# gaetanfacchinetti/DensityFlows.jl

Measured on AMD Instinct MI355X. Metric: forward+logdetJ Msamples/s, d=5 8-layer RealNVP, 1/2/4/8 MI355X, higher is better.
Workload: dtype f32

## Files before the change

densityflows.jl_amd/csrc/df_chain_impl.h:

```cpp
#pragma once

#include <hip/hip_runtime.h>

#include "df_kernels.h"

namespace df {

typedef float f32x4 __attribute__((ext_vector_type(4)));

#ifndef DF_WAVES_PER_EU
#define DF_WAVES_PER_EU(HT) ((HT) <= 4 ? 4 : 2)
#endif

namespace impl {

__device__ __forceinline__ float relu(float x) {
    return __int_as_float(__builtin_elementwise_max(__float_as_int(x), 0));
}

__device__ __forceinline__ float tanh_fast(float x) {
    const float x2 = x * x;
    const float n = fmaf(fmaf(fmaf(fmaf(1.587199e-8f, x2, 2.2332108e-5f), x2, 0.0035974074f), x2, 0.1346604f), x2, 1.0f);
    const float d =
        fmaf(fmaf(fmaf(fmaf(8.7767893e-7f, x2, 0.0003453992f), x2, 0.026262015f), x2, 0.4679937f), x2, 1.0f);
    return (x2 < 66.f) ? x * (n / d) : (x > 0.f ? 1.f : (x < 0.f ? -1.f : x));
}

__device__ __forceinline__ float sigmoid_fast(float x) {
    const float t = expf(-fabsf(x));
    const float y = (x >= 0.f) ? 1.f / (1.f + t) : t / (1.f + t);
    return (x > 40.f) ? 1.f : ((x < -80.f) ? 0.f : y);
}

__device__ __noinline__ float act_fn(int act, float x) {
    switch (act) {
        case DF_ACT_IDENTITY: return x;
        case DF_ACT_RELU: return relu(x);
        case DF_ACT_TANH: return tanh_fast(x);
        case DF_ACT_SIGMOID: return sigmoid_fast(x);
        case DF_ACT_SOFTPLUS: return log1pf(expf(-fabsf(x))) + ((x > 0.f) ? x : 0.f);
        case DF_ACT_LOGCOSH: {
            float y = -2.f * x;
            float sp = log1pf(expf(-fabsf(y))) + ((y > 0.f) ? y : 0.f);
            return (x + sp) - 0.6931471805599453f;
        }
        case DF_ACT_LEAKYRELU: return (x > 0.f) ? x : 0.01f * x;
        case DF_ACT_ELU: return (x > 0.f) ? x : expm1f(x);
        case DF_ACT_SWISH: {
            float t = expf(-fabsf(x));
            float sg = (x >= 0.f) ? 1.f / (1.f + t) : t / (1.f + t);
            return x * sg;
        }
        default: return x;
    }
}

__device__ __forceinline__ f32x4 mfma4(float a, float b, f32x4 c) {
    return __builtin_amdgcn_mfma_f32_16x16x4f32(a, b, c, 0, 0, 0);
}

__device__ __forceinline__ f32x4 lds4(const uint8_t* p) { return *reinterpret_cast<const f32x4*>(p); }

struct Smem {
    const int32_t* tab;
    float* state;
};

struct Stager {
    uint8_t* base;
    int bytes;
    const int32_t* sched;
    int n;
    int idx;
    int cur;
    __device__ __forceinline__ uint8_t* buf() const { return base + ((idx & 1) ? bytes : 0); }
};

template <typename T>
__device__ __forceinline__ T cload(const T* p, int64_t i) {
    using CT = const __attribute__((address_space(4))) T;
    return *(const T*)(&((CT*)(uintptr_t)p)[i]);
}

__device__ __forceinline__ void dma_stage(const ChainArgs& a, int s, uint8_t* dst) {
    const DevStage st = cload(a.stages, s);
    const int wave = __builtin_amdgcn_readfirstlane(threadIdx.x >> 6), lane = threadIdx.x & 63;
    const uint8_t* src = a.blob + st.src_off;
    const int nchunk = st.bytes >> 10;
    for (int c = wave; c < nchunk; c += kWavesPerBlock) {
        __builtin_amdgcn_global_load_lds(reinterpret_cast<const void*>(src + (c << 10) + lane * 16),
                                         (__attribute__((address_space(3))) void*)(dst + (c << 10)),
                                         16, 0, 0);
    }
}

__device__ __forceinline__ void stager_start(Stager& sg, const ChainArgs& a) {
    sg.idx = -1;
    sg.cur = -1;
    if (sg.n > 0) dma_stage(a, cload(sg.sched, 0), sg.base);
}

__device__ __forceinline__ void ensure_stage(int s, Stager& sg, const ChainArgs& a) {
    if (s == sg.cur) return;
#ifdef DF_EXP_NOSYNC
    if (sg.cur >= 0) { sg.cur = s; return; }
#endif
    const int nidx = sg.idx + 1;
    asm volatile("s_waitcnt vmcnt(0)" ::: "memory");
    __syncthreads();
    sg.idx = nidx;
    sg.cur = s;
    if (nidx >= sg.n || cload(sg.sched, nidx) != s) {
        const DevStage st = cload(a.stages, s);
        const f32x4* src = reinterpret_cast<const f32x4*>(a.blob + st.src_off);
        f32x4* dst = reinterpret_cast<f32x4*>(sg.buf());
        for (int i = threadIdx.x; i < (st.bytes >> 4); i += kBlockThreads) dst[i] = src[i];
        __syncthreads();
        sg.n = 0;
        return;
    }
    if (nidx + 1 < sg.n) dma_stage(a, cload(sg.sched, nidx + 1), sg.base + (((nidx + 1) & 1) ? sg.bytes : 0));
}

constexpr int out_tiles(int HT) { return HT < 2 ? HT : 2; }

template <int HT, int T, bool OUTV>
struct NetRegs {
    f32x4 h[T][HT];
    f32x4 acc[T][HT];
    f32x4 out[T][OUTV ? 1 : out_tiles(HT)];
};

template <int HT, int T>
__device__ __forceinline__ void dense_mfma(const ChainArgs& a, const DevDense& D, const int32_t* feat,
                                           Stager& sg, const Smem& sm, const int (&rowoff)[T],
                                           f32x4 (&h)[T][HT], f32x4 (&acc)[T][HT]) {
    const int lane = threadIdx.x & 63;
    const int g = lane >> 4;
    constexpr int MG = (T == 1) ? 2 : 1;
#pragma unroll
    for (int tt = 0; tt < T; ++tt)
#pragma unroll
        for (int m = 0; m < HT; ++m) acc[tt][m] = f32x4{0.f, 0.f, 0.f, 0.f};

    for (int c = 0; c < D.n_chunks; ++c) {
        const DevChunk C = a.chunks[D.chunk0 + c];
        ensure_stage(C.stage, sg, a);
        const uint8_t* base = sg.buf() + C.lds_off + lane * 16;
        if (D.in_kind == IN_STATE) {
#pragma unroll
            for (int kq = 0; kq < kMaxState / 16; ++kq) {
                if (kq >= C.kq_begin && kq < C.kq_end) {
                    float xin[T][4];
#pragma unroll
                    for (int r = 0; r < 4; ++r) {
                        const int s = 4 * kq + r;
                        if (s < D.ks) {
                            const int slot = feat[4 * s + g];
#pragma unroll
                            for (int tt = 0; tt < T; ++tt) xin[tt][r] = sm.state[rowoff[tt] + slot];
                        } else {
#pragma unroll
                            for (int tt = 0; tt < T; ++tt) xin[tt][r] = 0.f;
                        }
                    }
                    const uint8_t* bq = base + (kq - C.kq_begin) * D.mt * 1024;
                    if (HT >= 8 && D.mt == HT) {
                        constexpr int MB = HT < 4 ? HT : 4;
                        const int rmax = D.ks - 4 * kq;
#pragma unroll
                        for (int m0 = 0; m0 < HT; m0 += MB) {
                            f32x4 w[MB];
#pragma unroll
                            for (int mm = 0; mm < MB; ++mm) w[mm] = lds4(bq + (m0 + mm) * 1024);
#pragma unroll
                            for (int r = 0; r < 4; ++r)
                                if (r < rmax)
#pragma unroll
                                    for (int mm = 0; mm < MB; ++mm)
#pragma unroll
                                        for (int tt = 0; tt < T; ++tt)
                                            acc[tt][m0 + mm] = mfma4(w[mm][r], xin[tt][r], acc[tt][m0 + mm]);
                        }
                        continue;
                    }
#pragma unroll
                    for (int m0 = 0; m0 < HT; m0 += MG) {
                        if (m0 < D.mt) {
                            f32x4 w[MG];
#pragma unroll
                            for (int mm = 0; mm < MG; ++mm)
                                w[mm] = (m0 + mm < D.mt) ? lds4(bq + (m0 + mm) * 1024) : f32x4{0, 0, 0, 0};
#pragma unroll
                            for (int r = 0; r < 4; ++r) {
                                if (4 * kq + r < D.ks) {
#pragma unroll
                                    for (int mm = 0; mm < MG; ++mm)
                                        if (m0 + mm < HT && m0 + mm < D.mt)
#pragma unroll
                                            for (int tt = 0; tt < T; ++tt)
                                                acc[tt][m0 + mm] = mfma4(w[mm][r], xin[tt][r], acc[tt][m0 + mm]);
                                }
                            }
                        }
                    }
                }
            }
        } else if (D.mt == HT && C.kq_begin == 0 && C.kq_end == HT) {
            constexpr int MB = HT < 4 ? HT : 4;
#pragma unroll
            for (int m0 = 0; m0 < HT; m0 += MB) {
                f32x4 w[2][MB];
#pragma unroll
                for (int mm = 0; mm < MB; ++mm) w[0][mm] = lds4(base + (m0 + mm) * 1024);
#pragma unroll
                for (int kq = 0; kq < HT; ++kq) {
                    const int cb = kq & 1;
                    if (kq + 1 < HT) {
#pragma unroll
                        for (int mm = 0; mm < MB; ++mm)
                            w[cb ^ 1][mm] = lds4(base + ((kq + 1) * HT + m0 + mm) * 1024);
                    }
#pragma unroll
                    for (int r = 0; r < 4; ++r)
#pragma unroll
                        for (int mm = 0; mm < MB; ++mm)
#pragma unroll
                            for (int tt = 0; tt < T; ++tt)
                                acc[tt][m0 + mm] = mfma4(w[cb][mm][r], h[tt][kq][r], acc[tt][m0 + mm]);
                }
            }
        } else if (HT >= 8 && D.mt <= 2) {
            const int kb = C.kq_begin, ke = C.kq_end;
#pragma unroll
            for (int kq = 0; kq < HT; ++kq) {
                if (kq >= kb && kq < ke) {
                    const uint8_t* bq = base + (kq - kb) * D.mt * 1024;
                    const f32x4 w0 = lds4(bq);
                    if (D.mt == 2) {
                        const f32x4 w1 = lds4(bq + 1024);
#pragma unroll
                        for (int r = 0; r < 4; ++r)
#pragma unroll
                            for (int tt = 0; tt < T; ++tt) {
                                acc[tt][0] = mfma4(w0[r], h[tt][kq][r], acc[tt][0]);
                                acc[tt][1] = mfma4(w1[r], h[tt][kq][r], acc[tt][1]);
                            }
                    } else {
#pragma unroll
                        for (int r = 0; r < 4; ++r)
#pragma unroll
                            for (int tt = 0; tt < T; ++tt) acc[tt][0] = mfma4(w0[r], h[tt][kq][r], acc[tt][0]);
                    }
                }
            }
        } else if (D.mt == HT) {
            constexpr int MB = HT < 4 ? HT : 4;
            const int kb = C.kq_begin, ke = C.kq_end;
#pragma unroll
            for (int kq = 0; kq < HT; ++kq) {
                if (kq >= kb && kq < ke) {
                    const uint8_t* bq = base + (kq - kb) * HT * 1024;
                    f32x4 w[2][MB];
#pragma unroll
                    for (int mm = 0; mm < MB; ++mm) w[0][mm] = lds4(bq + mm * 1024);
#pragma unroll
                    for (int m0 = 0; m0 < HT; m0 += MB) {
                        const int cb = (m0 / MB) & 1;
                        if (m0 + MB < HT) {
#pragma unroll
                            for (int mm = 0; mm < MB; ++mm) w[cb ^ 1][mm] = lds4(bq + (m0 + MB + mm) * 1024);
                        }
#pragma unroll
                        for (int r = 0; r < 4; ++r)
#pragma unroll
                            for (int mm = 0; mm < MB; ++mm)
#pragma unroll
                                for (int tt = 0; tt < T; ++tt)
                                    acc[tt][m0 + mm] = mfma4(w[cb][mm][r], h[tt][kq][r], acc[tt][m0 + mm]);
                    }
                }
            }
        } else {
#pragma unroll
            for (int kq = 0; kq < HT; ++kq) {
                if (kq >= C.kq_begin && kq < C.kq_end) {
                    const uint8_t* bq = base + (kq - C.kq_begin) * D.mt * 1024;
#pragma unroll
                    for (int m0 = 0; m0 < HT; m0 += MG) {
                        if (m0 < D.mt) {
                            f32x4 w[MG];
#pragma unroll
                            for (int mm = 0; mm < MG; ++mm)
                                w[mm] = (m0 + mm < D.mt) ? lds4(bq + (m0 + mm) * 1024) : f32x4{0, 0, 0, 0};
#pragma unroll
                            for (int r = 0; r < 4; ++r)
#pragma unroll
                                for (int mm = 0; mm < MG; ++mm)
                                    if (m0 + mm < HT && m0 + mm < D.mt)
#pragma unroll
                                        for (int tt = 0; tt < T; ++tt)
                                            acc[tt][m0 + mm] = mfma4(w[mm][r], h[tt][kq][r], acc[tt][m0 + mm]);
                        }
                    }
                }
            }
        }
    }

    ensure_stage(D.bias_stage, sg, a);
    if (D.has_bias) {
#pragma unroll
        for (int m = 0; m < HT; ++m) {
            if (m < D.mt) {
                const f32x4 b = lds4(sg.buf() + D.bias_lds + ((16 * m + 4 * g) << 2));
#pragma unroll
                for (int tt = 0; tt < T; ++tt) acc[tt][m] = acc[tt][m] + b;
            }
        }
    }
    if (D.act == DF_ACT_RELU) {
#pragma unroll
        for (int m = 0; m < HT; ++m)
#pragma unroll
            for (int tt = 0; tt < T; ++tt)
#pragma unroll
                for (int r = 0; r < 4; ++r) acc[tt][m][r] = relu(acc[tt][m][r]);
    } else if (D.act != DF_ACT_IDENTITY) {
#ifndef DF_NO_GENERIC_ACT
#pragma unroll
        for (int m = 0; m < HT; ++m) {
            if (m < D.mt) {
#pragma unroll
                for (int tt = 0; tt < T; ++tt)
#pragma unroll
                    for (int r = 0; r < 4; ++r) acc[tt][m][r] = act_fn(D.act, acc[tt][m][r]);
            }
        }
#endif
    }
}

template <int HT, int T, bool OUTV>
__device__ __forceinline__ void eval_net(const ChainArgs& a, const DevLayer& L, int dense0, int ndense,
                                         Stager& sg, const Smem& sm, const int (&rowoff)[T],
                                         NetRegs<HT, T, OUTV>& R, float* hs = nullptr, int64_t gs = -1) {
    const int lane = threadIdx.x & 63;
    const int g = lane >> 4;
    const int32_t* feat = sm.tab + L.feat_tab;
    for (int k = 0; k < ndense; ++k) {
        const DevDense D = a.denses[dense0 + k];
        if (OUTV && k + 1 == ndense) {
            ensure_stage(D.w3_stage, sg, a);
            const uint8_t* w3 = sg.buf() + D.w3_lds;
            const int inp = 16 * D.kt_in;
            const float* b3 = reinterpret_cast<const float*>(w3) + D.n_out * inp;
#pragma unroll
            for (int o = 0; o < 4; ++o) {
                if (o < D.n_out) {
                    float p[T];
#pragma unroll
                    for (int tt = 0; tt < T; ++tt) p[tt] = 0.f;
#pragma unroll
                    for (int kq = 0; kq < HT; ++kq) {
                        if (kq < D.kt_in) {
                            f32x4 w = lds4(w3 + ((o * inp + 16 * kq + 4 * g) << 2));
#pragma unroll
                            for (int r = 0; r < 4; ++r)
#pragma unroll
                                for (int tt = 0; tt < T; ++tt) p[tt] = __builtin_fmaf(w[r], R.h[tt][kq][r], p[tt]);
                        }
                    }
#pragma unroll
                    for (int tt = 0; tt < T; ++tt) {
                        p[tt] += __shfl_xor(p[tt], 16);
                        p[tt] += __shfl_xor(p[tt], 32);
                        float v = p[tt];
                        if (D.has_bias) v = v + b3[o];
                        R.out[tt][0][o] = (D.act == DF_ACT_IDENTITY) ? v : act_fn(D.act, v);
                    }
                } else {
#pragma unroll
                    for (int tt = 0; tt < T; ++tt) R.out[tt][0][o] = 0.f;
                }
            }
            return;
        }
        dense_mfma<HT, T>(a, D, feat, sg, sm, rowoff, R.h, R.acc);
        if (k + 1 == ndense) {
            if constexpr (!OUTV) {
#pragma unroll
                for (int tt = 0; tt < T; ++tt)
#pragma unroll
                    for (int m = 0; m < out_tiles(HT); ++m) R.out[tt][m] = R.acc[tt][m];
            }
        } else {
#pragma unroll
            for (int tt = 0; tt < T; ++tt)
#pragma unroll
                for (int m = 0; m < HT; ++m) R.h[tt][m] = R.acc[tt][m];
            if (hs && gs >= 0) {
                float* dst = hs + ((int64_t)k * a.batch + gs) * a.hsave_w + 4 * g;
#pragma unroll
                for (int m = 0; m < HT; ++m)
                    if (m < D.mt) *reinterpret_cast<f32x4*>(dst + 16 * m) = R.acc[0][m];
            }
        }
    }
}

__device__ __forceinline__ float sel4(const f32x4 v, int i) {
    float r = v[0];
    r = (i == 1) ? v[1] : r;
    r = (i == 2) ? v[2] : r;
    r = (i == 3) ? v[3] : r;
    return r;
}

enum Phase { PH_S_FWD, PH_T_FWD, PH_T_BWD, PH_S_BWD };

template <int HT, int T, bool OUTV, int PH>
__device__ __forceinline__ void couple_phase(const NetRegs<HT, T, OUTV>& R, const DevLayer& L, const Smem& sm,
                                             const int (&rowoff)[T], float (&ssum)[T]) {
    const int g = (threadIdx.x & 63) >> 4;
// ... 281 lines not shown
```

densityflows.jl_amd/csrc/df_uniform_impl.h:

```cpp
#pragma once

#include <type_traits>

#include "df_chain_impl.h"

namespace df {
namespace uni {


using impl::lds4;
using impl::mfma4;
using impl::Stager;

__device__ __forceinline__ float relu_fast(float x) {
    return __int_as_float(__builtin_elementwise_max(__float_as_int(x), 0));
}

__device__ __forceinline__ float xgroup_sum(float p) {
    auto a = __builtin_amdgcn_permlane16_swap(__float_as_uint(p), __float_as_uint(p), false, false);
    const float q = __uint_as_float(a[0]) + __uint_as_float(a[1]);
    auto b = __builtin_amdgcn_permlane32_swap(__float_as_uint(q), __float_as_uint(q), false, false);
    return __uint_as_float(b[0]) + __uint_as_float(b[1]);
}

// ... 168 lines not shown
        }
        auto c = __builtin_amdgcn_permlane32_swap(__float_as_uint(A), __float_as_uint(Bv), false, false);
        y[t] = (__uint_as_float(c[0]) + __uint_as_float(c[1])) + bo;
    }
}

template <int NO>
__device__ __forceinline__ float group_row_sum(float y) {
    float s = y;
    if constexpr (NO > 1) {
        auto a = __builtin_amdgcn_permlane16_swap(__float_as_uint(y), __float_as_uint(y), false, false);
        s = s + __uint_as_float(a[1]);
    }
    if constexpr (NO > 2) {
        auto b = __builtin_amdgcn_permlane32_swap(__float_as_uint(y), __float_as_uint(y), false, false);
        const float y2 = __uint_as_float(b[1]);
        s = s + y2;
        if constexpr (NO > 3) {
            auto c = __builtin_amdgcn_permlane16_swap(__float_as_uint(y2), __float_as_uint(y2), false, false);
            s = s + __uint_as_float(c[1]);
        }
    }
    return s;
}

template <int HT, int TT, bool RELU>
__device__ __forceinline__ void out_mfma(const uint8_t* buf, const UNet& N, const f32x4 (&h)[TT][HT],
                                         f32x4 (&out)[TT][2]) {
    const int lane = threadIdx.x & 63, g = lane >> 4;
    const uint8_t* wb = buf + N.off_out + lane * 16;
    const int mt = (N.n_out + 15) >> 4;
#pragma unroll
    for (int t = 0; t < TT; ++t) out[t][0] = out[t][1] = f32x4{0.f, 0.f, 0.f, 0.f};
#pragma unroll
    for (int kq = 0; kq < HT; ++kq) {
        const f32x4 w0 = lds4(wb + (kq * mt + 0) * 1024);
#pragma unroll
        for (int r = 0; r < 4; ++r)
#pragma unroll
            for (int t = 0; t < TT; ++t) out[t][0] = mfma4(w0[r], h[t][kq][r], out[t][0]);
        if (mt > 1) {
            const f32x4 w1 = lds4(wb + (kq * mt + 1) * 1024);
#pragma unroll
            for (int r = 0; r < 4; ++r)
#pragma unroll
                for (int t = 0; t < TT; ++t) out[t][1] = mfma4(w1[r], h[t][kq][r], out[t][1]);
        }
    }
    const uint8_t* bb = buf + N.off_out + HT * mt * 1024;
#pragma unroll
    for (int m = 0; m < 2; ++m) {
        if (m < mt) {
            const f32x4 b = lds4(bb + ((16 * m + 4 * g) << 2));
#pragma unroll
            for (int t = 0; t < TT; ++t) {
                f32x4 v = out[t][m] + b;
                if (!RELU && N.act_out != DF_ACT_IDENTITY)
#pragma unroll
                    for (int r = 0; r < 4; ++r) v[r] = impl::act_fn(N.act_out, v[r]);
                out[t][m] = v;
            }
        }
    }
}

template <int PH>
__device__ __forceinline__ float couple1(float v, float y) {
    if (PH == impl::PH_S_FWD) return v * expf(y);
    if (PH == impl::PH_T_FWD) return v + y;
    if (PH == impl::PH_T_BWD) return v - y;
    return v * expf(-y);
}

template <int HT, int TT, bool OUTV, bool RELU, int PH, int NO = 0>
__device__ __forceinline__ void tail(const uint8_t* buf, const UNet& N, const ULayer& L, const int32_t* tab,
                                     float* state, const int (&ro)[TT], float (&sum)[TT], const f32x4 (&H)[TT][HT]) {
    const int g = (threadIdx.x & 63) >> 4;
    constexpr bool SPH = (PH == impl::PH_S_FWD || PH == impl::PH_S_BWD);
    const int32_t* af = tab + L.af_tab;
    const int n_af = (OUTV && NO > 0) ? NO : L.n_af;
#pragma unroll
    for (int t = 0; t < TT; ++t) sum[t] = 0.f;
#ifdef DF_EXP_NOTAIL
    if (true) {
#pragma unroll
        for (int t = 0; t < TT; ++t) {
            float acc = 0.f;
#pragma unroll
            for (int m = 0; m < HT; ++m) acc += H[t][m][0];
            asm volatile("" ::"v"(acc));
        }
        return;
    }
#endif
    if constexpr (OUTV && NO > 0) {
        float y[TT];
        out_valu_t<HT, TT, NO>(buf, N, H, y);
        const int slot = af[g < NO ? g : 0];
#pragma unroll
        for (int t = 0; t < TT; ++t) {
            if (g < NO) state[ro[t] + slot] = couple1<PH>(state[ro[t] + slot], y[t]);
            if (SPH) sum[t] = group_row_sum<NO>(y[t]);
        }
    } else if constexpr (OUTV) {
        f32x4 o[TT];
        out_valu<HT, TT, RELU, NO>(buf, N, H, o);
        const int slot = (g < n_af) ? af[g] : 0;
#pragma unroll
        for (int t = 0; t < TT; ++t) {
            const float y = impl::sel4(o[t], g);
            if (g < n_af) state[ro[t] + slot] = couple1<PH>(state[ro[t] + slot], y);
            if (SPH) {
                float s_ = o[t][0];
#pragma unroll
                for (int oo = 1; oo < 4; ++oo)
                    if (oo < n_af) s_ = s_ + o[t][oo];
                sum[t] = s_;
            }
        }
    } else {
        f32x4 o[TT][2];
        out_mfma<HT, TT, RELU>(buf, N, H, o);
#pragma unroll
        for (int t = 0; t < TT; ++t) {
            float p = 0.f;
#pragma unroll
            for (int m = 0; m < 2; ++m)
#pragma unroll
                for (int r = 0; r < 4; ++r) {
                    const int oo = 16 * m + 4 * g + r;
                    if (oo < L.n_af) {
                        const int slot = af[oo];
                        const float y = o[t][m][r];
                        state[ro[t] + slot] = couple1<PH>(state[ro[t] + slot], y);
                        if (SPH) p = p + y;
                    }
                }
            if (SPH) sum[t] = xgroup_sum(p);
        }
    }
}

typedef __bf16 bf16x8 __attribute__((ext_vector_type(8)));

__device__ __forceinline__ f32x4 mfma_bf(const bf16x8& a, const bf16x8& b, f32x4 c) {
    return __builtin_amdgcn_mfma_f32_16x16x32_bf16(a, b, c, 0, 0, 0);
}

typedef __bf16 bf16x2 __attribute__((ext_vector_type(2)));
#ifndef DF_SPLIT_DOT2
#define DF_SPLIT_DOT2 1
#endif
template <int S>
__device__ __forceinline__ float split_rem(bf16x2 h, float x) {
#if DF_SPLIT_DOT2 == 2
    const uint32_t u = __builtin_bit_cast(uint32_t, h);
    const float hi = __uint_as_float(S == 0 ? (u << 16) : (u & 0xffff0000u));
    float r;
    asm("v_sub_f32 %0, %1, %2" : "=v"(r) : "v"(x), "v"(hi));
    return r;
#elif DF_SPLIT_DOT2
    uint32_t c;
    if (S == 0) asm("v_mov_b32 %0, 0xbf80" : "=v"(c));
    else c = 0xbf800000u;
    return __builtin_amdgcn_fdot2_f32_bf16(h, __builtin_bit_cast(bf16x2, c), x, false);
#else
    return x - (float)h[S];
#endif
}

__device__ __forceinline__ void split2(float a, float b, bf16x2& p0, bf16x2& p1, bf16x2& p2) {
    p0 = bf16x2{(__bf16)a, (__bf16)b};
    const float ra = split_rem<0>(p0, a), rb = split_rem<1>(p0, b);
    p1 = bf16x2{(__bf16)ra, (__bf16)rb};
    p2 = bf16x2{(__bf16)split_rem<0>(p1, ra), (__bf16)split_rem<1>(p1, rb)};
}

__device__ __forceinline__ void split8(const float (&v)[8], bf16x8& p0, bf16x8& p1, bf16x8& p2) {
#pragma unroll
    for (int e = 0; e < 8; e += 2) {
        bf16x2 h, m, l;
        split2(v[e], v[e + 1], h, m, l);
        p0[e] = h[0]; p0[e + 1] = h[1];
        p1[e] = m[0]; p1[e + 1] = m[1];
        p2[e] = l[0]; p2[e + 1] = l[1];
    }
}

#ifndef DF_SPLIT_MREM
#define DF_SPLIT_MREM 1
#endif
typedef short short4v __attribute__((ext_vector_type(4)));
typedef __bf16 bf16x4v __attribute__((ext_vector_type(4)));

__device__ __forceinline__ short4v neg_eye() {
    const int i = threadIdx.x & 3;
    short4v p;
#pragma unroll
    for (int e = 0; e < 4; ++e) p[e] = (e == i) ? (short)0xbf80 : (short)0;
    return p;
}

__device__ __forceinline__ f32x4 mrem(short4v eye, bf16x4v h, f32x4 c) {
    return __builtin_amdgcn_mfma_f32_4x4x4bf16_1k(eye, __builtin_bit_cast(short4v, h), c, 0, 0, 0);
}

__device__ __forceinline__ void split8_mrem(short4v eye, const f32x4& a, const f32x4& b, bf16x8& p0, bf16x8& p1,
                                            bf16x8& p2) {
    bf16x4v h0, h1;
#pragma unroll
    for (int e = 0; e < 4; ++e) {
        h0[e] = (__bf16)a[e];
        h1[e] = (__bf16)b[e];
    }
    p0 = __builtin_shufflevector(h0, h1, 0, 1, 2, 3, 4, 5, 6, 7);
    const f32x4 ra = mrem(eye, h0, a), rb = mrem(eye, h1, b);
#pragma unroll
    for (int e = 0; e < 4; ++e) {
        h0[e] = (__bf16)ra[e];
        h1[e] = (__bf16)rb[e];
    }
    p1 = __builtin_shufflevector(h0, h1, 0, 1, 2, 3, 4, 5, 6, 7);
    const f32x4 sa = mrem(eye, h0, ra), sb = mrem(eye, h1, rb);
#pragma unroll
    for (int e = 0; e < 4; ++e) {
        h0[e] = (__bf16)sa[e];
        h1[e] = (__bf16)sb[e];
    }
    p2 = __builtin_shufflevector(h0, h1, 0, 1, 2, 3, 4, 5, 6, 7);
}

template <int HT, int TT>
__device__ __forceinline__ void dense_first_split(const uint8_t* buf, const UNet& N, const float (&xin)[TT][4],
                                                  f32x4 (&acc)[TT][HT]) {
    const int lane = threadIdx.x & 63;
    bf16x8 b[TT];
    const __bf16 z = (__bf16)0.f;
#pragma unroll
    for (int t = 0; t < TT; t += 2) {
        bf16x2 h, m, l;
        split2(xin[t][0], t + 1 < TT ? xin[t + 1][0] : 0.f, h, m, l);
        b[t] = bf16x8{h[0], m[0], h[0], l[0], m[0], h[0], z, z};
        if (t + 1 < TT) b[t + 1] = bf16x8{h[1], m[1], h[1], l[1], m[1], h[1], z, z};
    }
    const uint8_t* wb = buf + N.off_w0 + lane * 16;
#pragma unroll
    for (int m = 0; m < HT; ++m) {
        const bf16x8 w = *reinterpret_cast<const bf16x8*>(wb + m * 1024);
#pragma unroll
        for (int t = 0; t < TT; ++t) acc[t][m] = mfma_bf(w, b[t], f32x4{0.f, 0.f, 0.f, 0.f});
    }
}

template <int HT, int TT, bool BIAS = true, bool FENCE = false>
__device__ __forceinline__ void dense_hidden_split(const uint8_t* wb, const f32x4 (&in)[TT][HT],
                                                   f32x4 (&out)[TT][HT]) {
    const int lane = threadIdx.x & 63, g = lane >> 4;
    const uint8_t* bb = wb + (HT / 2) * HT * 3072;
    wb += lane * 16;
    const short4v eye = DF_SPLIT_MREM ? neg_eye() : short4v{0, 0, 0, 0};
#pragma unroll
    for (int m = 0; m < HT; ++m) {
        const f32x4 b = BIAS ? lds4(bb + ((16 * m + 4 * g) << 2)) : f32x4{0.f, 0.f, 0.f, 0.f};
#pragma unroll
        for (int t = 0; t < TT; ++t) out[t][m] = b;
    }
#pragma unroll
    for (int c = 0; c < HT / 2; ++c) {
        bf16x8 x[TT][3];
#pragma unroll
        for (int t = 0; t < TT; ++t) {
            const float v[8] = {in[t][2 * c][0],     in[t][2 * c][1],     in[t][2 * c][2],     in[t][2 * c][3],
                                in[t][2 * c + 1][0], in[t][2 * c + 1][1], in[t][2 * c + 1][2], in[t][2 * c + 1][3]};
#ifdef DF_DIAG_NOSPLIT
            for (int e = 0; e < 8; ++e) x[t][0][e] = (__bf16)v[e];
            x[t][1] = x[t][0];
            x[t][2] = x[t][0];
#else
            if constexpr (DF_SPLIT_MREM) split8_mrem(eye, in[t][2 * c], in[t][2 * c + 1], x[t][0], x[t][1], x[t][2]);
            else split8(v, x[t][0], x[t][1], x[t][2]);
#endif
        }
#pragma unroll
        for (int m = 0; m < HT; ++m) {
            const uint8_t* f = wb + (c * HT + m) * 3072;
            const bf16x8 w0 = *reinterpret_cast<const bf16x8*>(f);
            const bf16x8 w1 = *reinterpret_cast<const bf16x8*>(f + 1024);
            const bf16x8 w2 = *reinterpret_cast<const bf16x8*>(f + 2048);
#pragma unroll
            for (int t = 0; t < TT; ++t) {
                f32x4 a = out[t][m];
                a = mfma_bf(w2, x[t][0], a);
                a = mfma_bf(w1, x[t][1], a);
                a = mfma_bf(w0, x[t][2], a);
                a = mfma_bf(w1, x[t][0], a);
                a = mfma_bf(w0, x[t][1], a);
                out[t][m] = mfma_bf(w0, x[t][0], a);
            }
            if (FENCE) asm volatile("" ::: "memory");
        }
    }
}

template <int HT, int TT, bool OUTV, bool RELU, int PH, bool FAST = false, int NO = 0, bool SPLIT = false>
__device__ __forceinline__ void net_tiles(const uint8_t* buf, const UNet& N, const ULayer& L, const int32_t* tab,
                                          float* state, const int (&ro)[TT], float (&sum)[TT]) {
    const int lane = threadIdx.x & 63, g = lane >> 4;
    constexpr bool SPH = (PH == impl::PH_S_FWD || PH == impl::PH_S_BWD);
    if constexpr (SPLIT && FAST && HT >= 2) {
        float xin[TT][4];
        const int slot = tab[L.feat_tab + g];
#pragma unroll
        for (int t = 0; t < TT; ++t) xin[t][0] = state[ro[t] + slot];
        f32x4 A[TT][HT], B[TT][HT];
        dense_first_split<HT, TT>(buf, N, xin, A);
        bias_act<HT, TT, true>(buf, DF_ACT_RELU, A, false);
        dense_hidden_split<HT, TT>(buf + N.off_h, A, B);
        bias_act<HT, TT, true>(buf, DF_ACT_RELU, B, false);
        tail<HT, TT, OUTV, RELU, PH, NO>(buf, N, L, tab, state, ro, sum, B);
        return;
    }
    float xin[TT][4];
    const int32_t* feat = tab + L.feat_tab;
    constexpr int KS = FAST ? 1 : 0;
    const int ks = FAST ? 1 : N.ks;
#pragma unroll
    for (int r = 0; r < 4; ++r) {
        const int slot = (r < ks) ? feat[4 * r + g] : 0;
#pragma unroll
        for (int t = 0; t < TT; ++t) xin[t][r] = (r < ks) ? state[ro[t] + slot] : 0.f;
    }

    f32x4 A[TT][HT], B[TT][HT];
    dense_first<HT, TT, KS>(buf, N, xin, A);
    bias_act<HT, TT, RELU>(buf + N.off_b0, N.act0, A, FAST ? false : !N.fold0);
    if (FAST || N.nh == 1) {
        dense_hidden<HT, TT>(buf + N.off_h, A, B);
        bias_act<HT, TT, RELU>(buf + N.off_h + HT * HT * 1024, N.acth, B);
        tail<HT, TT, OUTV, RELU, PH, NO>(buf, N, L, tab, state, ro, sum, B);
        return;
    }
    bool in_a = true;
    for (int k = 0; k < N.nh; k += 2) {
        dense_hidden<HT, TT>(buf + N.off_h + k * N.hstride, A, B);
        bias_act<HT, TT, RELU>(buf + N.off_h + k * N.hstride + HT * HT * 1024, N.acth, B);
        in_a = false;
        if (k + 1 < N.nh) {
            dense_hidden<HT, TT>(buf + N.off_h + (k + 1) * N.hstride, B, A);
            bias_act<HT, TT, RELU>(buf + N.off_h + (k + 1) * N.hstride + HT * HT * 1024, N.acth, A);
            in_a = true;
        }
    }
    if (in_a) tail<HT, TT, OUTV, RELU, PH, NO>(buf, N, L, tab, state, ro, sum, A);
    else tail<HT, TT, OUTV, RELU, PH, NO>(buf, N, L, tab, state, ro, sum, B);
}

template <int HT, int TT, bool RELU, bool FWDP, int NO>
__device__ __forceinline__ void net_pair_tiles(const uint8_t* buf, const ULayer& L, const int32_t* tab, float* state,
                                               const int (&ro)[TT], float (&ssum)[TT]) {
    const int lane = threadIdx.x & 63, g = lane >> 4;
    float xin[TT][4];
    const int slot_in = tab[L.feat_tab + g];
#pragma unroll
    for (int t = 0; t < TT; ++t) xin[t][0] = state[ro[t] + slot_in];
    f32x4 As[TT][HT], At[TT][HT], Bs[TT][HT], Bt[TT][HT];
    dense_first<HT, TT, 1>(buf, L.s, xin, As);
    dense_first<HT, TT, 1>(buf, L.t, xin, At);
    bias_act<HT, TT, RELU>(buf + L.s.off_b0, L.s.act0, As, false);
    bias_act<HT, TT, RELU>(buf + L.t.off_b0, L.t.act0, At, false);
    dense_hidden<HT, TT>(buf + L.s.off_h, As, Bs);
    dense_hidden<HT, TT>(buf + L.t.off_h, At, Bt);
    bias_act<HT, TT, RELU>(buf + L.s.off_h + HT * HT * 1024, L.s.acth, Bs);
    bias_act<HT, TT, RELU>(buf + L.t.off_h + HT * HT * 1024, L.t.acth, Bt);
    float ys[TT], yt[TT];
    out_valu_t<HT, TT, NO>(buf, L.s, Bs, ys);
    out_valu_t<HT, TT, NO>(buf, L.t, Bt, yt);
    const int slot = tab[L.af_tab + (g < NO ? g : 0)];
#pragma unroll
    for (int t = 0; t < TT; ++t) {
        if (g < NO) {
            float v = state[ro[t] + slot];
            if (FWDP) {
                v = v * expf(ys[t]);
                v = v + yt[t];
            } else {
                v = v - yt[t];
                v = v * expf(-ys[t]);
            }
            state[ro[t] + slot] = v;
        }
        ssum[t] = group_row_sum<NO>(ys[t]);
    }
}

}

#ifndef DF_UNI_WAVES
#define DF_UNI_WAVES 4
#endif
#ifndef DF_FAST_WAVES
#define DF_FAST_WAVES 4
#endif

template <int HT, int MODE, bool OUTV, bool RELU, bool FAST = false, bool SPLIT = false>
__global__ void __launch_bounds__(kBlockThreads, FAST ? DF_FAST_WAVES : DF_UNI_WAVES)
uniform_kernel(ChainArgs a) {
    using namespace uni;
    constexpr bool FWD = (MODE == MODE_FWD || MODE == MODE_FWD_INPLACE);
    constexpr bool WANT_LDJ = (MODE != MODE_FWD_INPLACE);

    extern __shared__ __attribute__((aligned(16))) uint8_t smem[];
    const int stage_area = a.stage_bytes * a.n_stage_bufs;
    int32_t* tab = reinterpret_cast<int32_t*>(smem + stage_area);
    float* state = reinterpret_cast<float*>(smem + stage_area + a.tab_bytes);

    ClockStamp clk;
    clk.begin(a);
#ifdef DF_PHASE_STAMPS
    uint64_t ph[16] = {};
#define DF_PH(i) do { if (blockIdx.x == 0 && threadIdx.x == 0) ph[i] = __builtin_amdgcn_s_memtime(); } while (0)
#else
#define DF_PH(i) do {} while (0)
#endif
    DF_PH(0);
    const int tid = threadIdx.x;
    const int lane = tid & 63, wave = tid >> 6;
    const int g = lane >> 4, j = lane & 15;
    const int d = a.d, n = a.n, stride = a.stride, nd = n + d;
    const int nt = a.tiles;
    const int S = kWavesPerBlock * 16 * nt;
    const int cA = nd + 1, cE = nd + 2;
    const int64_t s0 = (int64_t)blockIdx.x * S;
    const int nvalid = (int)((a.batch - s0) < S ? (a.batch - s0) : S);

    Stager sg;
    sg.base = smem;
    sg.bytes = a.stage_bytes;
    sg.sched = FWD ? a.sched_fwd : a.sched_bwd;
    sg.n = FWD ? a.n_sched_fwd : a.n_sched_bwd;
    impl::stager_start(sg, a);

    float* tabf = reinterpret_cast<float*>(tab);
    constexpr int kRowMax = 8;
    const bool fast_copy = d <= kRowMax && n <= kRowMax && a.n_par <= kBlockThreads && a.tab_ints <= 4 * kBlockThreads;
    auto row_init = [&](int smp) {
        for (int c = nd; c < stride; ++c) state[smp * stride + c] = (c == nd + 3) ? 1.f : 0.f;
    };
    auto theta_in = [&](float v, float lo, float hi) {
        const float diff = hi - lo;
        return (diff == 0.f) ? 0.f : (v - lo) / diff;
    };
    if (fast_copy) {
        const int n_tab = a.tab_ints, n_par = a.n_par;
        int tv[4];
#pragma unroll
        for (int u = 0; u < 4; ++u) {
            const int i = tid + u * kBlockThreads;
            tv[u] = i < n_tab ? a.tables[i] : 0;
        }
        const float pv = tid < n_par ? a.params[tid] : 0.f;
        const bool norm_th = a.tmin != nullptr;
        const float blo = (norm_th && lane < n) ? a.tmin[lane] : 0.f;
        const float bhi = (norm_th && lane < n) ? a.tmax[lane] : 0.f;
        const int smp = tid;
        const bool valid = smp < nvalid;
        float zr[kRowMax], tr[kRowMax];
#pragma unroll
        for (int c = 0; c < kRowMax; ++c)
            if (c < d) zr[c] = valid ? a.zin[(s0 + smp) * d + c] : 0.f;
#pragma unroll
        for (int c = 0; c < kRowMax; ++c)
            if (c < n) tr[c] = valid ? a.theta[(s0 + smp) * n + c] : 0.f;
#pragma unroll
        for (int u = 0; u < 4; ++u) {
            const int i = tid + u * kBlockThreads;
            if (i < n_tab) tab[i] = tv[u];
        }
        if (tid < n_par) tabf[n_tab + tid] = pv;
#pragma unroll
        for (int c = 0; c < kRowMax; ++c)
            if (c < n) {
                const float lo = __shfl(blo, c), hi = __shfl(bhi, c);
                if (smp < S) state[smp * stride + c] = (norm_th && valid) ? theta_in(tr[c], lo, hi) : tr[c];
            }
        if (smp < S) {
#pragma unroll
            for (int c = 0; c < kRowMax; ++c)
                if (c < d) state[smp * stride + n + c] = zr[c];
            row_init(smp);
        }
        for (int i = tid + kBlockThreads * d; i < S * d; i += kBlockThreads) {
            const int r = i / d, c = i - r * d;
            state[r * stride + n + c] = r < nvalid ? a.zin[(s0 + r) * d + c] : 0.f;
        }
        for (int i = tid + kBlockThreads * n; i < S * n; i += kBlockThreads) {
            const int r = i / n, c = i - r * n;
            float v = 0.f;
            if (r < nvalid) {
                v = a.theta[(s0 + r) * n + c];
                if (norm_th) v = theta_in(v, a.tmin[c], a.tmax[c]);
            }
            state[r * stride + c] = v;
        }
        for (int r = tid + kBlockThreads; r < S; r += kBlockThreads) row_init(r);
    } else {
        for (int i = tid; i < a.tab_ints; i += kBlockThreads) tab[i] = a.tables[i];
        for (int i = tid; i < S * d; i += kBlockThreads) {
            const int smp = i / d, c = i - smp * d;
            float v = 0.f;
            if (smp < nvalid) v = a.zin[(s0 + smp) * d + c];
            state[smp * stride + n + c] = v;
        }
        for (int i = tid; i < S * n; i += kBlockThreads) {
            const int smp = i / n, c = i - smp * n;
            float v = 0.f;
            if (smp < nvalid) {
                v = a.theta[(s0 + smp) * n + c];
                if (a.tmin) v = theta_in(v, a.tmin[c], a.tmax[c]);
            }
            state[smp * stride + c] = v;
        }
        for (int i = tid; i < S; i += kBlockThreads) row_init(i);
    }
    DF_PH(1);
    DF_PH(2);
    DF_PH(3);
    __syncthreads();
    DF_PH(4);

    const int row0 = ((wave * nt) * 16 + j) * stride;
#ifdef DF_NO_PAIR
    constexpr bool no_pair = true;
#else
    constexpr bool no_pair = false;
#endif
    const int tstep = 16 * stride;
    bool have_acc = false;

    auto ldj_update = [&](int ro, float l, bool first_in_elem, bool last_in_elem) {
        if (!WANT_LDJ || g != 0) return;
        const float e = first_in_elem ? l : state[ro + cE] + l;
        state[ro + cE] = e;
        if (last_in_elem) state[ro + cA] = have_acc ? state[ro + cA] + e : e;
    };

    for (int it = 0; it < a.n_layers; ++it) {
        const int li = FWD ? it : a.n_layers - 1 - it;
        using CULayer = const __attribute__((address_space(4))) ULayer;
#ifdef DF_PHASE_STAMPS
        const ULayer L = *(const ULayer*)(&((CULayer*)(uintptr_t)a.ulayers)[li]);
        asm volatile("s_waitcnt lgkmcnt(0)" ::: "memory");
        if (it == 1) DF_PH(13);
#else
        const ULayer& L = *(const ULayer*)(&((CULayer*)(uintptr_t)a.ulayers)[li]);
#endif
        const int kind = L.kind;
        const bool first_in_elem = FWD ? L.elem_start : L.elem_end;
        const bool last_in_elem = FWD ? L.elem_end : L.elem_start;
        if (kind == DF_LAYER_NORM) {
            const float al = L.alpha, be = L.beta, delta = be - al;
            auto norm = [&](const auto* xmn) {
                const auto* xmx = xmn + d;
                for (int tt = 0; tt < nt; ++tt) {
                    const int ro = row0 + tt * tstep;
                    for (int i = g; i < d; i += 4) {
                        const float lo = xmn[i], hi = xmx[i], xd = hi - lo;
                        float v = state[ro + n + i];
                        if (FWD) v = ((xd * v - al * hi) + be * lo) / delta;
                        else v = (be * (v - lo) + al * (hi - v)) / xd;
                        state[ro + n + i] = v;
                    }
                    ldj_update(ro, FWD ? L.ldj_const : -L.ldj_const, first_in_elem, last_in_elem);
                }
            };
            if (fast_copy) norm(tabf + a.tab_ints + L.norm_off);
            else norm(a.params + L.norm_off);
        } else {
            const bool rnvp = (kind == DF_LAYER_RNVP);
            constexpr int kTT = FAST ? kFastTileGroup : kUniformTileGroup;
            auto tiles_loop = [&](const UNet& N, auto ph_tag, auto no_tag, bool sphase, float sign) {
                constexpr int PH = decltype(ph_tag)::value;
                constexpr int NO = decltype(no_tag)::value;
                const uint8_t* buf = sg.buf();
                for (int tt = 0; tt < nt; tt += kTT) {
                    int ro[kTT];
                    float ssum[kTT];
                    int r0 = row0;
                    if constexpr (SPLIT) asm volatile("" : "+v"(r0));
#pragma unroll
                    for (int t = 0; t < kTT; ++t) ro[t] = r0 + (tt + t) * tstep;
                    net_tiles<HT, kTT, OUTV, RELU, PH, FAST, NO, SPLIT>(buf, N, L, tab, state, ro, ssum);
#pragma unroll
                    for (int t = 0; t < kTT; ++t) {
                        if (sphase) ldj_update(ro[t], sign * ssum[t], first_in_elem, last_in_elem);
                        else if (!rnvp) ldj_update(ro[t], 0.f, first_in_elem, last_in_elem);
                    }
                }
            };
            auto run_net = [&](const UNet& N, auto ph_tag, bool sphase, float sign) {
                impl::ensure_stage(N.stage, sg, a);
                if constexpr (FAST && OUTV) {
                    switch (N.n_out) {
                        case 1: tiles_loop(N, ph_tag, std::integral_constant<int, 1>{}, sphase, sign); break;
                        case 2: tiles_loop(N, ph_tag, std::integral_constant<int, 2>{}, sphase, sign); break;
                        case 3: tiles_loop(N, ph_tag, std::integral_constant<int, 3>{}, sphase, sign); break;
                        default: tiles_loop(N, ph_tag, std::integral_constant<int, 4>{}, sphase, sign); break;
                    }
                } else {
                    tiles_loop(N, ph_tag, std::integral_constant<int, 0>{}, sphase, sign);
                }
            };
            using PSF = std::integral_constant<int, impl::PH_S_FWD>;
            using PTF = std::integral_constant<int, impl::PH_T_FWD>;
            using PTB = std::integral_constant<int, impl::PH_T_BWD>;
            using PSB = std::integral_constant<int, impl::PH_S_BWD>;
            bool paired = false;
            if constexpr (FAST && OUTV && !SPLIT && HT <= 2) {
                if (rnvp && L.s.stage == L.t.stage && L.s.n_out == L.t.n_out && !no_pair) {
                    impl::ensure_stage(L.s.stage, sg, a);
                    auto pair_loop = [&](auto no_tag) {
                        constexpr int NO = decltype(no_tag)::value;
                        const uint8_t* buf = sg.buf();
                        for (int tt = 0; tt < nt; tt += kTT) {
                            int ro[kTT];
                            float ssum[kTT];
#pragma unroll
                            for (int t = 0; t < kTT; ++t) ro[t] = row0 + (tt + t) * tstep;
                            net_pair_tiles<HT, kTT, RELU, FWD, NO>(buf, L, tab, state, ro, ssum);
#pragma unroll
                            for (int t = 0; t < kTT; ++t)
                                ldj_update(ro[t], FWD ? ssum[t] : -ssum[t], first_in_elem, last_in_elem);
                        }
                    };
                    switch (L.s.n_out) {
                        case 1: pair_loop(std::integral_constant<int, 1>{}); break;
                        case 2: pair_loop(std::integral_constant<int, 2>{}); break;
                        case 3: pair_loop(std::integral_constant<int, 3>{}); break;
                        default: pair_loop(std::integral_constant<int, 4>{}); break;
                    }
                    paired = true;
                }
            }
            if (paired) {
            } else if (FWD) {
#ifdef DF_PHASE_STAMPS
                if (it == 1) DF_PH(11);
#endif
                if (rnvp) run_net(L.s, PSF{}, true, 1.f);
#ifdef DF_PHASE_STAMPS
                if (it == 1) DF_PH(12);
#endif
                run_net(L.t, PTF{}, false, 1.f);
            } else {
                run_net(L.t, PTB{}, false, 1.f);
                if (rnvp) run_net(L.s, PSB{}, true, -1.f);
            }
        }
        have_acc = have_acc || last_in_elem;
#ifdef DF_PHASE_STAMPS
        if (it == 0) DF_PH(5);
        if (it == 1) DF_PH(6);
        if (it == 2) DF_PH(7);
        if (it == 3) DF_PH(8);
#endif
        if (!FWD && a.snap) {
            float* dst = a.snap + (int64_t)li * a.batch * d;
            for (int tt = 0; tt < nt; ++tt) {
                const int smp = (wave * nt + tt) * 16 + j;
                if (smp < nvalid)
                    for (int i = g; i < d; i += 4) dst[(s0 + smp) * d + i] = state[row0 + tt * tstep + n + i];
            }
        }
    }

    asm volatile("s_waitcnt vmcnt(0)" ::: "memory");
    if (MODE == MODE_LOGPDF) {
        double part = 0.0;
        if (g == 0) {
            for (int tt = 0; tt < nt; ++tt) {
                const int ro = row0 + tt * tstep;
                const int smp = (wave * nt + tt) * 16 + j;
                float q = 0.f;
                for (int i = 0; i < d; ++i) {
                    const float zz = state[ro + n + i];
                    q = q + zz * zz;
                }
                const float lp = (a.c0 - q / 2.f) + state[ro + cA];
                if (smp < nvalid) {
                    if (a.lp_out) a.lp_out[s0 + smp] = lp;
                    part += (double)lp;
                }
            }
        }
        if (a.partial) {
#pragma unroll
            for (int off = 32; off >= 1; off >>= 1) part += __shfl_xor(part, off);
            __syncthreads();
            double* red = reinterpret_cast<double*>(smem);
            if (lane == 0) red[wave] = part;
            __syncthreads();
            if (tid == 0) {
                double s = 0.0;
                for (int w = 0; w < kWavesPerBlock; ++w) s += red[w];
                a.partial[blockIdx.x] = s;
            }
        }
        if (!a.xout) {
            clk.end(a);
            return;
        }
    }
    __syncthreads();
    for (int i = tid; i < S * d; i += kBlockThreads) {
        const int smp = i / d, c = i - smp * d;
        if (smp < nvalid) a.xout[(s0 + smp) * d + c] = state[smp * stride + n + c];
    }
    if (WANT_LDJ && MODE != MODE_LOGPDF && a.ldj_out) {
        for (int i = tid; i < nvalid; i += kBlockThreads) a.ldj_out[s0 + i] = state[i * stride + cA];
    }
    DF_PH(9);
#ifdef DF_PHASE_STAMPS
    asm volatile("s_waitcnt vmcnt(0)" ::: "memory");
    DF_PH(10);
    if (blockIdx.x == 0 && threadIdx.x == 0) {
#pragma unroll
        for (int i = 1; i < 14; ++i) a.xout[i] = (float)(ph[i] - ph[0]);
    }
#endif
#undef DF_PH
    clk.end(a);
}

template <int HT, bool RELU, bool FAST = false, bool SPLIT = false>
void* uniform_kernel_ptr_r(int mode, bool outv) {
#define DF_U(M) (outv ? reinterpret_cast<void*>(&uniform_kernel<HT, M, true, RELU, FAST, SPLIT>) \
                      : reinterpret_cast<void*>(&uniform_kernel<HT, M, false, RELU, FAST, SPLIT>))
    switch (mode) {
        case MODE_FWD: return DF_U(MODE_FWD);
        case MODE_FWD_INPLACE: return DF_U(MODE_FWD_INPLACE);
        case MODE_BWD: return DF_U(MODE_BWD);
        default: return DF_U(MODE_LOGPDF);
    }
#undef DF_U
}

template <int HT>
void* uniform_kernel_ptr(int mode, int variant) {
    const bool outv = variant & 1;
    if constexpr (HT >= 2) {
        if ((variant & 8) && (variant & 4) && outv) return uniform_kernel_ptr_r<HT, true, true, true>(mode, true);
    }
    if (variant & 8) return nullptr;
    if (variant & 4) return uniform_kernel_ptr_r<HT, true, true>(mode, outv);
    return (variant & 2) ? uniform_kernel_ptr_r<HT, true>(mode, outv) : uniform_kernel_ptr_r<HT, false>(mode, outv);
}

template <int HT>
hipError_t launch_uniform_ht(int mode, int variant, const ChainArgs& a, unsigned grid, size_t lds, hipStream_t st) {
    void* args[] = {const_cast<ChainArgs*>(&a)};
    return hipLaunchKernel(uniform_kernel_ptr<HT>(mode, variant), dim3(grid), dim3(kBlockThreads), args, lds, st);
}

template <int HT>
hipError_t set_uniform_lds_limit_ht(size_t lds) {
    for (int mode = 0; mode < 4; ++mode)
        for (int v = 0; v < 16; ++v) {
            void* k = uniform_kernel_ptr<HT>(mode, v);
            if (!k) continue;
            hipError_t e = hipFuncSetAttribute(k,
                                               hipFuncAttributeMaxDynamicSharedMemorySize, (int)lds);
            if (e != hipSuccess) return e;
        }
    return hipSuccess;
}

template <int HT>
hipError_t uniform_occupancy_ht(int mode, int variant, size_t lds, int* blocks) {
    return hipOccupancyMaxActiveBlocksPerMultiprocessor(blocks, uniform_kernel_ptr<HT>(mode, variant), kBlockThreads,
                                                        lds);
}

}
```

Before: 1618.

## Software-pipeline LDS weight loads in split-bf16 MLP path with double buffering

Adds a prefetching variant of the split-precision MLP path. Hidden-layer and output-layer weights are read from LDS one step ahead into double-buffered registers, with sched_barrier fences and explicit waitcnt calls. The aim is to hide LDS latency behind the MFMA and FMA work. It also pins lane-derived offsets in VGPRs via inline asm, in the DMA staging and in the norm/snapshot paths, to steer register allocation. The cost is higher register pressure, and the hand-placed fences may limit the compiler's own scheduling.

Result: faster. 1656 (median of 6 runs) (+2.3%).

```diff
diff --git a/densityflows.jl_amd/csrc/df_chain_impl.h b/densityflows.jl_amd/csrc/df_chain_impl.h
--- a/densityflows.jl_amd/csrc/df_chain_impl.h
+++ b/densityflows.jl_amd/csrc/df_chain_impl.h
@@ -82,24 +82,30 @@
     return *(const T*)(&((CT*)(uintptr_t)p)[i]);
 }
 
+template <bool LANE_LOCAL = false>
 __device__ __forceinline__ void dma_stage(const ChainArgs& a, int s, uint8_t* dst) {
     const DevStage st = cload(a.stages, s);
     const int wave = __builtin_amdgcn_readfirstlane(threadIdx.x >> 6), lane = threadIdx.x & 63;
+    uint32_t loff = lane * 16;
+    if constexpr (LANE_LOCAL) asm volatile("" : "+v"(loff));
     const uint8_t* src = a.blob + st.src_off;
     const int nchunk = st.bytes >> 10;
     for (int c = wave; c < nchunk; c += kWavesPerBlock) {
-        __builtin_amdgcn_global_load_lds(reinterpret_cast<const void*>(src + (c << 10) + lane * 16),
+        const uint8_t* from = LANE_LOCAL ? src + (c << 10) + loff : src + (c << 10) + lane * 16;
+        __builtin_amdgcn_global_load_lds(reinterpret_cast<const void*>(from),
                                          (__attribute__((address_space(3))) void*)(dst + (c << 10)),
                                          16, 0, 0);
     }
 }
 
+template <bool LANE_LOCAL = false>
 __device__ __forceinline__ void stager_start(Stager& sg, const ChainArgs& a) {
     sg.idx = -1;
     sg.cur = -1;
-    if (sg.n > 0) dma_stage(a, cload(sg.sched, 0), sg.base);
-}
-
+    if (sg.n > 0) dma_stage<LANE_LOCAL>(a, cload(sg.sched, 0), sg.base);
+}
+
+template <bool LANE_LOCAL = false>
 __device__ __forceinline__ void ensure_stage(int s, Stager& sg, const ChainArgs& a) {
     if (s == sg.cur) return;
 #ifdef DF_EXP_NOSYNC
@@ -119,7 +125,7 @@
         sg.n = 0;
         return;
     }
-    if (nidx + 1 < sg.n) dma_stage(a, cload(sg.sched, nidx + 1), sg.base + (((nidx + 1) & 1) ? sg.bytes : 0));
+    if (nidx + 1 < sg.n) dma_stage<LANE_LOCAL>(a, cload(sg.sched, nidx + 1), sg.base + (((nidx + 1) & 1) ? sg.bytes : 0));
 }
 
 constexpr int out_tiles(int HT) { return HT < 2 ? HT : 2; }
diff --git a/densityflows.jl_amd/csrc/df_uniform_impl.h b/densityflows.jl_amd/csrc/df_uniform_impl.h
--- a/densityflows.jl_amd/csrc/df_uniform_impl.h
+++ b/densityflows.jl_amd/csrc/df_uniform_impl.h
@@ -494,11 +494,190 @@
     }
 }
 
+#ifndef DF_SPLIT_PREFETCH
+#define DF_SPLIT_PREFETCH 1
+#endif
+
+__device__ __forceinline__ void sched_fence() { __builtin_amdgcn_sched_barrier(0); }
+
+__device__ __forceinline__ void lds_wait0() { __builtin_amdgcn_s_waitcnt(0xc07f); }
+
+struct SplitStep {
+    bf16x8 w0, w1, w2;
+    f32x4 b;
+};
+
+template <int HT, bool BIAS>
+__device__ __forceinline__ void split_step_request(const uint8_t* wl, const uint8_t* bl, int s, SplitStep& f) {
+    if (s >= (HT / 2) * HT) return;
+    const uint8_t* p = wl + s * 3072;
+    f.w0 = *reinterpret_cast<const bf16x8*>(p);
+    f.w1 = *reinterpret_cast<const bf16x8*>(p + 1024);
+    f.w2 = *reinterpret_cast<const bf16x8*>(p + 2048);
+    if (BIAS && s < HT) f.b = lds4(bl + (s << 6));
+}
+
+template <int HT, int TT, bool BIAS = true>
+__device__ __forceinline__ void dense_hidden_split_pf(const uint8_t* wb, int lane, const f32x4 (&in)[TT][HT],
+                                                      f32x4 (&out)[TT][HT], const SplitStep& f0) {
+    const int g = lane >> 4;
+    const uint8_t* bl = wb + (HT / 2) * HT * 3072 + (g << 4);
+    const uint8_t* wl = wb + lane * 16;
+    const short4v eye = neg_eye();
+    SplitStep f[2];
+    f[0] = f0;
+    bf16x8 x[TT][3];
+#pragma unroll
+    for (int s = 0; s < (HT / 2) * HT; ++s) {
+        const int c = s / HT, m = s % HT;
+        if (m == 0) {
+#pragma unroll
+            for (int t = 0; t < TT; ++t) split8_mrem(eye, in[t][2 * c], in[t][2 * c + 1], x[t][0], x[t][1], x[t][2]);
+        }
+        constexpr int NS = (HT / 2) * HT;
+        const bool late = (m == HT - 1) && (s + 1 < NS);
+        sched_fence();
+        lds_wait0();
+        if (!late) split_step_request<HT, BIAS>(wl, bl, s + 1, f[(s + 1) & 1]);
+        sched_fence();
+        const SplitStep& w = f[s & 1];
+#pragma unroll
+        for (int t = 0; t < TT; ++t) {
+            f32x4 a = c == 0 ? (BIAS ? w.b : f32x4{0.f, 0.f, 0.f, 0.f}) : out[t][m];
+            a = mfma_bf(w.w2, x[t][0], a);
+            a = mfma_bf(w.w1, x[t][1], a);
+            a = mfma_bf(w.w0, x[t][2], a);
+            a = mfma_bf(w.w1, x[t][0], a);
+            a = mfma_bf(w.w0, x[t][1], a);
+            out[t][m] = mfma_bf(w.w0, x[t][0], a);
+        }
+        if (late) {
+#pragma unroll
+            for (int t = 0; t < TT; ++t) asm volatile("" : "+v"(out[t][m]));
+            sched_fence();
+            split_step_request<HT, BIAS>(wl, bl, s + 1, f[(s + 1) & 1]);
+        }
+    }
+}
+
+template <int HT, int TT>
+__device__ __forceinline__ void dense_first_split_pf(const bf16x8 (&w)[HT], const float (&xin)[TT][4],
+                                                     f32x4 (&acc)[TT][HT]) {
+    bf16x8 b[TT];
+    const __bf16 z = (__bf16)0.f;
+#pragma unroll
+    for (int t = 0; t < TT; t += 2) {
+        bf16x2 h, m, l;
+        split2(xin[t][0], t + 1 < TT ? xin[t + 1][0] : 0.f, h, m, l);
+        b[t] = bf16x8{h[0], m[0], h[0], l[0], m[0], h[0], z, z};
+        if (t + 1 < TT) b[t + 1] = bf16x8{h[1], m[1], h[1], l[1], m[1], h[1], z, z};
+    }
+#pragma unroll
+    for (int m = 0; m < HT; ++m)
+#pragma unroll
+        for (int t = 0; t < TT; ++t) acc[t][m] = mfma_bf(w[m], b[t], f32x4{0.f, 0.f, 0.f, 0.f});
+}
+
+template <int HT, int NO>
+__device__ __forceinline__ void out_row_request(const uint8_t* w3g, int oo, f32x4 (&w)[HT]) {
+    if (oo >= NO) return;
+#pragma unroll
+    for (int kq = 0; kq < HT; ++kq) w[kq] = lds4(w3g + ((oo * 16 * HT + 16 * kq) << 2));
+}
+
+template <int HT, int TT, int NO>
+__device__ __forceinline__ void out_valu_t_pf(const uint8_t* w3g, const f32x4 (&w0)[HT], float bo,
+                                              const f32x4 (&h)[TT][HT], const float* state, const int (&ro)[TT],
+                                              const int& aslot, float (&v)[TT], float (&y)[TT]) {
+    static_assert(NO >= 1 && NO <= 4, "FAST tails: 1..4 outputs");
+    float p[TT][4];
+#pragma unroll
+    for (int t = 0; t < TT; ++t)
+#pragma unroll
+        for (int oo = 0; oo < 4; ++oo) p[t][oo] = 0.f;
+    f32x4 w[2][HT];
+#pragma unroll
+    for (int kq = 0; kq < HT; ++kq) w[0][kq] = w0[kq];
+#pragma unroll
+    for (int oo = 0; oo < NO; ++oo) {
+        sched_fence();
+        lds_wait0();
+        if (oo == 0) {
+#pragma unroll
+            for (int t = 0; t < TT; ++t) v[t] = state[ro[t] + aslot];
+        }
+        out_row_request<HT, NO>(w3g, oo + 1, w[(oo + 1) & 1]);
+        sched_fence();
+#pragma unroll
+        for (int kq = 0; kq < HT; ++kq)
+#pragma unroll
+            for (int r = 0; r < 4; ++r)
+#pragma unroll
+                for (int t = 0; t < TT; ++t) p[t][oo] = __builtin_fmaf(w[oo & 1][kq][r], h[t][kq][r], p[t][oo]);
+#pragma unroll
+        for (int t = 0; t < TT; ++t) asm volatile("" : "+v"(p[t][oo]));
+    }
+#pragma unroll
+    for (int t = 0; t < TT; ++t) {
+        auto a = __builtin_amdgcn_permlane16_swap(__float_as_uint(p[t][0]), __float_as_uint(p[t][1]), false, false);
+        const float A = __uint_as_float(a[0]) + __uint_as_float(a[1]);
+        float Bv = 0.f;
+        if constexpr (NO > 2) {
+            auto b = __builtin_amdgcn_permlane16_swap(__float_as_uint(p[t][2]), __float_as_uint(p[t][3]), false, false);
+            Bv = __uint_as_float(b[0]) + __uint_as_float(b[1]);
+        }
+        auto c = __builtin_amdgcn_permlane32_swap(__float_as_uint(A), __float_as_uint(Bv), false, false);
+        y[t] = (__uint_as_float(c[0]) + __uint_as_float(c[1])) + bo;
+    }
+}
+
 template <int HT, int TT, bool OUTV, bool RELU, int PH, bool FAST = false, int NO = 0, bool SPLIT = false>
 __device__ __forceinline__ void net_tiles(const uint8_t* buf, const UNet& N, const ULayer& L, const int32_t* tab,
                                           float* state, const int (&ro)[TT], float (&sum)[TT]) {
     const int lane = threadIdx.x & 63, g = lane >> 4;
     constexpr bool SPH = (PH == impl::PH_S_FWD || PH == impl::PH_S_BWD);
+#if DF_SPLIT_PREFETCH && !defined(DF_EXP_NOTAIL) && !defined(DF_DIAG_NOSPLIT)
+    if constexpr (SPLIT && FAST && HT >= 2 && OUTV && NO > 0) {
+        int tx = threadIdx.x;
+        asm volatile("" : "+v"(tx));
+        const int lane = tx & 63, g = lane >> 4;
+        const int off_out = N.off_out, af_tab = L.af_tab;
+        asm volatile("" ::"s"(off_out), "s"(af_tab));
+        const int slot = tab[L.feat_tab + g];
+        bf16x8 w0[HT];
+#pragma unroll
+        for (int m = 0; m < HT; ++m) w0[m] = *reinterpret_cast<const bf16x8*>(buf + N.off_w0 + lane * 16 + m * 1024);
+        sched_fence();
+        lds_wait0();
+        float xin[TT][4];
+#pragma unroll
+        for (int t = 0; t < TT; ++t) xin[t][0] = state[ro[t] + slot];
+        const uint8_t* wh = buf + N.off_h;
+        SplitStep f0;
+        split_step_request<HT, true>(wh + lane * 16, wh + (HT / 2) * HT * 3072 + (g << 4), 0, f0);
+        sched_fence();
+        f32x4 A[TT][HT], B[TT][HT];
+        dense_first_split_pf<HT, TT>(w0, xin, A);
+        bias_act<HT, TT, true>(buf, DF_ACT_RELU, A, false);
+        dense_hidden_split_pf<HT, TT>(wh, lane, A, B, f0);
+        const uint8_t* w3g = buf + off_out + (g << 4);
+        sched_fence();
+        f32x4 wo[HT];
+        out_row_request<HT, NO>(w3g, 0, wo);
+        const float bo = reinterpret_cast<const float*>(buf + off_out)[NO * 16 * HT + (g < NO ? g : 0)];
+        const int aslot = tab[af_tab + (g < NO ? g : 0)];
+        sched_fence();
+        bias_act<HT, TT, true>(buf, DF_ACT_RELU, B, false);
+        float v[TT], y[TT];
+        out_valu_t_pf<HT, TT, NO>(w3g, wo, bo, B, state, ro, aslot, v, y);
+#pragma unroll
+        for (int t = 0; t < TT; ++t) {
+            if (g < NO) state[ro[t] + aslot] = couple1<PH>(v[t], y[t]);
+            sum[t] = SPH ? group_row_sum<NO>(y[t]) : 0.f;
+        }
+        return;
+    }
+#endif
     if constexpr (SPLIT && FAST && HT >= 2) {
         float xin[TT][4];
         const int slot = tab[L.feat_tab + g];
@@ -630,7 +809,8 @@
     sg.bytes = a.stage_bytes;
     sg.sched = FWD ? a.sched_fwd : a.sched_bwd;
     sg.n = FWD ? a.n_sched_fwd : a.n_sched_bwd;
-    impl::stager_start(sg, a);
+    constexpr bool kLaneLocalDma = SPLIT && DF_SPLIT_PREFETCH;
+    impl::stager_start<kLaneLocalDma>(sg, a);
 
     float* tabf = reinterpret_cast<float*>(tab);
     constexpr int kRowMax = 8;
@@ -749,13 +929,22 @@
         const int kind = L.kind;
         const bool first_in_elem = FWD ? L.elem_start : L.elem_end;
         const bool last_in_elem = FWD ? L.elem_end : L.elem_start;
+        int gl = g, jl = j, wavel = wave, row0l = row0;
+        if constexpr (kLaneLocalDma) {
+            if (kind == DF_LAYER_NORM || (!FWD && a.snap)) {
+                int tx = tid;
+                asm volatile("" : "+v"(tx));
+                gl = (tx & 63) >> 4, jl = tx & 15, wavel = tx >> 6;
+                row0l = ((wavel * nt) * 16 + jl) * stride;
+            }
+        }
         if (kind == DF_LAYER_NORM) {
             const float al = L.alpha, be = L.beta, delta = be - al;
             auto norm = [&](const auto* xmn) {
                 const auto* xmx = xmn + d;
                 for (int tt = 0; tt < nt; ++tt) {
-                    const int ro = row0 + tt * tstep;
-                    for (int i = g; i < d; i += 4) {
+                    const int ro = row0l + tt * tstep;
+                    for (int i = gl; i < d; i += 4) {
                         const float lo = xmn[i], hi = xmx[i], xd = hi - lo;
                         float v = state[ro + n + i];
                         if (FWD) v = ((xd * v - al * hi) + be * lo) / delta;
@@ -790,7 +979,7 @@
                 }
             };
             auto run_net = [&](const UNet& N, auto ph_tag, bool sphase, float sign) {
-                impl::ensure_stage(N.stage, sg, a);
+                impl::ensure_stage<kLaneLocalDma>(N.stage, sg, a);
                 if constexpr (FAST && OUTV) {
                     switch (N.n_out) {
                         case 1: tiles_loop(N, ph_tag, std::integral_constant<int, 1>{}, sphase, sign); break;
@@ -858,9 +1047,9 @@
         if (!FWD && a.snap) {
             float* dst = a.snap + (int64_t)li * a.batch * d;
             for (int tt = 0; tt < nt; ++tt) {
-                const int smp = (wave * nt + tt) * 16 + j;
+                const int smp = (wavel * nt + tt) * 16 + jl;
                 if (smp < nvalid)
-                    for (int i = g; i < d; i += 4) dst[(s0 + smp) * d + i] = state[row0 + tt * tstep + n + i];
+                    for (int i = gl; i < d; i += 4) dst[(s0 + smp) * d + i] = state[row0l + tt * tstep + n + i];
             }
         }
     }
```
